# natir/br

Measured on AMD Instinct MI355X. Metric: corrected Gbases/sec at k=19, 10 kb ONT-error reads, higher is better.
Workload: dtype u64 k-mers / 1-bit set

## Files before the change

br_amd/csrc/brx_partbuild.hip:

```cpp
#include "brx_internal.hpp"
#include "brx_index.hpp"

#include <stdlib.h>
#include <string.h>

namespace brx {
uint64_t scan_tmp_bytes(uint32_t n);
int exclusive_scan_lens(const uint32_t *d_lens, uint32_t n, uint64_t *d_tmp, uint64_t *d_out_offsets,
                        unsigned long long *d_total, hipStream_t s);
}

using namespace brx;

namespace {

constexpr int F_BITS = 12;
constexpr int MAX_LEVELS = 4;
constexpr int MAX_DIGIT_BITS = 9;
static_assert(MAX_DIGIT_BITS <= 9, "the digit scans of the partition passes are written for at most 512 digits");

struct Plan {
    int k, nbits, nlev;
    int bits[MAX_LEVELS];
    int rem_in[MAX_LEVELS];
// ... 102 lines not shown
    const unsigned long long lo = x * R;
    unsigned long long hi = lo + R;
    if (hi > n_items)
        hi = n_items;
    return {lo + j, hi, (G - x + 7ull) >> 3};
}

struct L1Args {
    const uint8_t *bases;
    const uint64_t *offsets;
    uint32_t n_reads;
    uint64_t total;
    uint32_t n_items;
    int k, nbits, bits;
    uint32_t *matrix;
    const uint64_t *pos;
    uint32_t *keys_out;
    uint64_t out_cap;
};

__device__ __forceinline__ void l1_prepare(const L1Args &a, uint32_t item, uint32_t *pk, uint32_t *bnd, uint32_t *sh_r0,
                                           uint32_t &n_here, bool search)
{
    const uint64_t off0 = a.offsets[0];
    const uint64_t g0 = (uint64_t)item * L1_TILE;
    const uint64_t left = a.total - g0;
    n_here = (uint32_t)(left < L1_TILE ? left : L1_TILE);
    const uint32_t win = n_here + (uint32_t)a.k + 32u;
    pack_window(a.bases + off0, a.total, g0, win, pk);
    for (uint32_t w = threadIdx.x; w < BND_WORDS; w += 256)
        bnd[w] = 0;
// ... 37 lines not shown

struct L1Next {
    uint4 q0, q1;
    uint64_t off;
    uint32_t m[(1u << MAX_DIGIT_BITS) / 256u];
};

__device__ __forceinline__ uint32_t l1_window_words(const L1Args &a, uint32_t item, uint32_t &n_here)
{
    const uint64_t left = a.total - (uint64_t)item * L1_TILE;
    n_here = (uint32_t)(left < L1_TILE ? left : L1_TILE);
    return (n_here + (uint32_t)a.k + 32u + 15u) / 16u;
}

template <bool ROW>
__device__ __forceinline__ void l1_fetch(const L1Args &a, uint32_t item, uint32_t r_first, L1Next &nx)
{
    const uint64_t off0 = a.offsets[0];
    const uint8_t *bases = a.bases + off0;
    const uint64_t g0 = (uint64_t)item * L1_TILE;
    uint32_t n_here;
    const uint32_t nwords = l1_window_words(a, item, n_here);
    const uint64_t p0 = g0 + 16ull * threadIdx.x, p1 = p0 + 16ull * 256ull;
    nx.q0 = make_uint4(0, 0, 0, 0);
    nx.q1 = make_uint4(0, 0, 0, 0);
    if (threadIdx.x < nwords && p0 + 16 <= a.total)
        __builtin_memcpy(&nx.q0, bases + p0, 16);
    if (256u + threadIdx.x < nwords && p1 + 16 <= a.total)
        __builtin_memcpy(&nx.q1, bases + p1, 16);
    const uint32_t r = r_first + threadIdx.x;
    nx.off = a.offsets[r <= a.n_reads ? r : a.n_reads] - off0;
    if (ROW) {
        const uint32_t B = 1u << a.bits;
#pragma unroll
        for (uint32_t q = 0; q < (1u << MAX_DIGIT_BITS) / 256u; q++) {
            const uint32_t b = threadIdx.x + 256u * q;
            nx.m[q] = b < B ? a.matrix[(uint64_t)item * B + b] : 0u;
        }
    }
}

__device__ __forceinline__ uint32_t l1_pack16(const L1Args &a, const uint4 &q, uint64_t p)
{
    uint32_t v[4] = {q.x, q.y, q.z, q.w};
    if (p + 16 > a.total) {
        const uint8_t *bases = a.bases + a.offsets[0];
        v[0] = v[1] = v[2] = v[3] = 0;
        for (uint32_t j = 0; j < 16; j++)
            if (p + j < a.total)
                v[j >> 2] |= (uint32_t)bases[p + j] << (8u * (j & 3u));
    }
    return (pack4(v[0]) << 24) | (pack4(v[1]) << 16) | (pack4(v[2]) << 8) | pack4(v[3]);
}

__device__ __forceinline__ void l1_consume(const L1Args &a, uint32_t item, const L1Next &nx, uint32_t *pk, uint32_t *bnd, uint32_t *sh_r0,
                                           uint32_t &n_here, bool first)
{
    const uint64_t off0 = a.offsets[0];
    const uint64_t g0 = (uint64_t)item * L1_TILE;
    const uint32_t nwords = l1_window_words(a, item, n_here);
    if (threadIdx.x < nwords)
        pk[threadIdx.x] = l1_pack16(a, nx.q0, g0 + 16ull * threadIdx.x);
    if (256u + threadIdx.x < nwords)
        pk[256u + threadIdx.x] = l1_pack16(a, nx.q1, g0 + 16ull * (256u + threadIdx.x));
    for (uint32_t w = threadIdx.x; w < BND_WORDS; w += 256)
        bnd[w] = 0;
    if (threadIdx.x == 0 && !first) {
        sh_r0[0] += sh_r0[1];
        sh_r0[1] = 0;
    }
    __syncthreads();
    const uint64_t lim = g0 + n_here + (uint64_t)a.k;
    uint32_t before_next = 0;
    uint64_t o = nx.off;
    for (uint32_t r = sh_r0[0] + threadIdx.x; r <= a.n_reads; r += 256) {
        if (o >= lim)
            break;
        const uint32_t p = (uint32_t)(o - g0);
        atomicOr(&bnd[p >> 5], 1u << (p & 31u));
        before_next += o <= g0 + L1_TILE ? 1u : 0u;
        if (r + 256u <= a.n_reads)
            o = a.offsets[r + 256u] - off0;
    }
    if (before_next)
        atomicAdd(&sh_r0[1], before_next);
    __syncthreads();
}

__device__ __forceinline__ void l1_search(const L1Args &a, uint32_t item, uint32_t *sh_r0)
{
    if (threadIdx.x == 0) {
        const uint64_t off0 = a.offsets[0], g0 = (uint64_t)item * L1_TILE;
        uint32_t lo = 0, hi = a.n_reads + 1;
        while (lo < hi) {
            const uint32_t mid = lo + (hi - lo) / 2;
            if (a.offsets[mid] - off0 <= g0)
                lo = mid + 1;
            else
                hi = mid;
        }
        sh_r0[0] = lo;
        sh_r0[1] = 0;
    }
    __syncthreads();
}

__device__ __forceinline__ bool l1_valid(const uint32_t *bnd, uint32_t p, int k)
{
    const uint32_t q = p + 1u;
    const uint32_t w = q >> 5, sh = q & 31u;
    const uint64_t two = ((uint64_t)bnd[w + 1] << 32) | bnd[w];
    const uint32_t bits = (uint32_t)(two >> sh) & ((k > 1) ? ((1u << (k - 1)) - 1u) : 0u);
    return bits == 0u;
}

static_assert(L1_TILE == 256u * 16u, "l1_for_each_hash: 16 positions per thread");
template <int UNROLL = 4, typename F>
// ... 18 lines not shown
#pragma unroll UNROLL
    for (uint32_t j = 0; j < left; j++) {
        if ((vb & vmask) == 0ull)
            f(((popc64(fwd) & 1) ? rc : fwd) >> 1);
        const uint64_t b = next >> 62;
        next <<= 2;
        vb >>= 1;
        fwd = ((fwd << 2) | b) & mask;
        rc = (rc >> 2) | ((b ^ 2ull) << top);
    }
}

#ifndef BRX_L1HIST_WAVES
#define BRX_L1HIST_WAVES 1
#endif
__global__ __launch_bounds__(256, BRX_L1HIST_WAVES) void l1_hist_kernel(L1Args a)
{
    extern __shared__ uint32_t lds[];
    __shared__ uint32_t pk[PACK_WORDS];
    __shared__ uint32_t bnd[BND_WORDS];
    __shared__ uint32_t sh_r0[2];
    const uint32_t B = 1u << a.bits;
    const int shift = a.nbits - a.bits;
    uint32_t lo, hi;
    l1_range(a.n_items, lo, hi);
    if (lo >= hi)
        return;
    l1_search(a, lo, sh_r0);
    L1Next nx;
    l1_fetch<false>(a, lo, sh_r0[0], nx);
    for (uint32_t item = lo; item < hi; item++) {
        for (uint32_t b = threadIdx.x; b < B; b += 256)
            lds[b] = 0;
        uint32_t n_here;
        l1_consume(a, item, nx, pk, bnd, sh_r0, n_here, item == lo);
        if (item + 1 < hi)
            l1_fetch<false>(a, item + 1, sh_r0[0] + sh_r0[1], nx);
        l1_for_each_hash(pk, bnd, n_here, a.k, [&](uint64_t h) { atomicAdd(&lds[(uint32_t)(h >> shift)], 1u); });
        __syncthreads();
        for (uint32_t b = threadIdx.x; b < B; b += 256)
            a.matrix[(uint64_t)item * B + b] = lds[b];
        __syncthreads();
    }
}

__global__ __launch_bounds__(256) void col_scan_partial_kernel(const uint32_t *__restrict__ m, uint32_t n_items, uint32_t B, uint32_t CH,
                                                               uint64_t *__restrict__ part)
{
    const uint32_t chunk = blockIdx.x;
    const uint32_t lo = chunk * CH, hi = (lo + CH < n_items) ? lo + CH : n_items;
    for (uint32_t b = threadIdx.x; b < B; b += 256) {
        uint64_t sum = 0;
        for (uint32_t it = lo; it < hi; it++)
            sum += m[(uint64_t)it * B + b];
        part[(uint64_t)chunk * B + b] = sum;
    }
}

__global__ __launch_bounds__(256) void col_scan_columns_kernel(uint64_t *__restrict__ part, uint32_t n_chunks, uint32_t B,
                                                               uint64_t *__restrict__ coltot)
{
    __shared__ uint64_t wsum[4];
    const uint32_t b = blockIdx.x;
    const uint32_t per = (n_chunks + 255u) / 256u;
    const uint32_t c0 = threadIdx.x * per;
    uint64_t v[8];
    uint64_t mine = 0;
    for (uint32_t q = 0; q < per && q < 8u; q++) {
        const uint32_t c = c0 + q;
        v[q] = c < n_chunks ? part[(uint64_t)c * B + b] : 0;
        mine += v[q];
    }
    uint64_t incl = mine;
    for (int d = 1; d < 64; d <<= 1) {
        const uint64_t t = __shfl_up(incl, d);
        if ((threadIdx.x & 63) >= (unsigned)d)
            incl += t;
    }
    if ((threadIdx.x & 63) == 63)
        wsum[threadIdx.x >> 6] = incl;
    __syncthreads();
    uint64_t base = 0;
    for (uint32_t w = 0; w < (threadIdx.x >> 6); w++)
        base += wsum[w];
    uint64_t run = base + incl - mine;
    for (uint32_t q = 0; q < per && q < 8u; q++) {
        const uint32_t c = c0 + q;
        if (c < n_chunks)
            part[(uint64_t)c * B + b] = run;
        run += v[q];
    }
    if (threadIdx.x == 255)
        coltot[b] = base + incl;
}

__global__ __launch_bounds__(64) void col_scan_digits_kernel(const uint64_t *__restrict__ coltot, uint32_t B, uint64_t *__restrict__ coff,
                                                             unsigned long long *__restrict__ total)
{
    uint64_t carry = 0;
    for (uint32_t b0 = 0; b0 < B; b0 += 64) {
        const uint32_t b = b0 + threadIdx.x;
        const uint64_t v = b < B ? coltot[b] : 0;
        uint64_t incl = v;
        for (int d = 1; d < 64; d <<= 1) {
            const uint64_t t = __shfl_up(incl, d);
            if (threadIdx.x >= (unsigned)d)
                incl += t;
        }
        if (b < B)
            coff[b] = carry + incl - v;
        carry += __shfl(incl, 63);
    }
    if (threadIdx.x == 0) {
        coff[B] = carry;
        *total = carry;
    }
}

__global__ __launch_bounds__(256) void col_scan_positions_kernel(const uint32_t *__restrict__ m, uint32_t n_items, uint32_t B, uint32_t CH,
                                                                 const uint64_t *__restrict__ part, const uint64_t *__restrict__ coff,
                                                                 uint64_t *__restrict__ pos)
{
    const uint32_t chunk = blockIdx.x;
    const uint32_t lo = chunk * CH, hi = (lo + CH < n_items) ? lo + CH : n_items;
    for (uint32_t b = threadIdx.x; b < B; b += 256) {
        uint64_t run = part[(uint64_t)chunk * B + b] + coff[b];
        for (uint32_t it = lo; it < hi; it++) {
            pos[(uint64_t)it * B + b] = run;
            run += m[(uint64_t)it * B + b];
        }
    }
}

template <bool TABLE>
__global__ __launch_bounds__(256) void flat_insert_kernel(L1Args a, uint32_t *__restrict__ bits, uint64_t *__restrict__ lines,
                                                          uint32_t line_shift, uint32_t m, uint32_t w,
                                                          unsigned long long *__restrict__ n_new)
{
    __shared__ uint32_t pk[PACK_WORDS];
    __shared__ uint32_t bnd[BND_WORDS];
    __shared__ uint32_t sh_r0[2];
    uint32_t added = 0;
    uint32_t lo, hi;
    l1_range(a.n_items, lo, hi);
    for (uint32_t item = lo; item < hi; item++) {
// ... 7 lines not shown
                } else {
                    const uint64_t h = khash(kmer, a.k);
                    atomicOr(bits + (h >> 5), 1u << (h & 31u));
                }
            }
        __syncthreads();
    }
    if (TABLE) {
        for (int d = 32; d > 0; d >>= 1)
            added += __shfl_down(added, d);
        if ((threadIdx.x & 63) == 0 && added)
            atomicAdd(n_new, (unsigned long long)added);
    }
}

__device__ __forceinline__ void block_scan_bins(uint32_t B, const uint32_t *cntv, uint32_t *lofs, uint32_t *lcur, uint32_t *sh_wsum)
{
    const uint32_t BPT = (B + 255u) / 256u;
    uint32_t mine = 0;
    for (uint32_t q = 0; q < BPT; q++) {
        const uint32_t b = threadIdx.x * BPT + q;
        if (b < B)
            mine += cntv[b];
    }
    uint32_t incl = mine;
    for (int d = 1; d < 64; d <<= 1) {
        const uint32_t t = __shfl_up(incl, d);
        if ((threadIdx.x & 63) >= (unsigned)d)
            incl += t;
    }
    if ((threadIdx.x & 63) == 63)
        sh_wsum[threadIdx.x >> 6] = incl;
    __syncthreads();
    uint32_t wbase = 0;
    for (uint32_t w = 0; w < (threadIdx.x >> 6); w++)
        wbase += sh_wsum[w];
    uint32_t run = wbase + incl - mine;
    for (uint32_t q = 0; q < BPT; q++) {
        const uint32_t b = threadIdx.x * BPT + q;
        if (b < B) {
            lofs[b] = run;
            lcur[b] = run;
            run += cntv[b];
        }
    }
}

constexpr uint32_t L1_SECTOR = 8;
constexpr uint32_t L1_OWN = ((1u << MAX_DIGIT_BITS) + 255u) / 256u;

#ifndef BRX_L1SCAT_WAVES
#define BRX_L1SCAT_WAVES 5
#endif
__global__ __launch_bounds__(256, BRX_L1SCAT_WAVES) void l1_scatter_kernel(L1Args a)
{
    extern __shared__ __attribute__((aligned(16))) uint8_t lds_raw[];
    __shared__ uint32_t pk[PACK_WORDS];
    __shared__ uint32_t bnd[BND_WORDS];
    __shared__ uint32_t sh_r0[2];
    __shared__ uint32_t sh_wsum[4];
    const uint32_t T = L1_TILE;
    const uint32_t B = 1u << a.bits;
    uint32_t *stage_key = (uint32_t *)lds_raw;
    unsigned long long *gsm = (unsigned long long *)(stage_key + T);
    uint32_t *cntv = (uint32_t *)(gsm + B);
    uint32_t *lofs = cntv + B;
    uint32_t *lcur = lofs + B;
    const int shift = a.nbits - a.bits;
    const uint64_t child_mask = (1ull << shift) - 1ull;
    uint32_t lo, hi;
    l1_range(a.n_items, lo, hi);
    if (lo >= hi)
        return;
    for (uint32_t b = threadIdx.x; b < B; b += 256) {
        const unsigned long long p0 = a.pos[(uint64_t)lo * B + b];
        const unsigned long long ph = p0 & (L1_SECTOR - 1);
        gsm[b] = (p0 / L1_SECTOR) | (ph << 32) | (ph << 36);
    }
    uint32_t creg[L1_OWN][L1_SECTOR];
#pragma unroll
    for (uint32_t q = 0; q < L1_OWN; q++)
#pragma unroll
        for (uint32_t jj = 0; jj < L1_SECTOR; jj++)
            creg[q][jj] = 0;
    l1_search(a, lo, sh_r0);
    L1Next nx;
    l1_fetch<true>(a, lo, sh_r0[0], nx);
    for (uint32_t item = lo; item < hi; item++) {
#pragma unroll
        for (uint32_t q = 0; q < L1_OWN; q++)
            if (threadIdx.x + 256u * q < B)
                cntv[threadIdx.x + 256u * q] = nx.m[q];
        uint32_t n_here;
        l1_consume(a, item, nx, pk, bnd, sh_r0, n_here, item == lo);
        if (item + 1 < hi)
            l1_fetch<true>(a, item + 1, sh_r0[0] + sh_r0[1], nx);
        block_scan_bins(B, cntv, lofs, lcur, sh_wsum);
        __syncthreads();
        l1_for_each_hash<BRX_L1_UNROLL>(pk, bnd, n_here, a.k, [&](uint64_t h) {
            const uint32_t d = (uint32_t)(h >> shift);
            const uint32_t slot = atomicAdd(&lcur[d], 1u);
            stage_key[slot] = (uint32_t)(h & child_mask);
        });
        __syncthreads();
#pragma unroll
        for (uint32_t q = 0; q < L1_OWN; q++) {
            const uint32_t d = threadIdx.x + 256u * q;
            if (d < B) {
                const unsigned long long m = gsm[d];
                const uint32_t n = cntv[d], base = lofs[d];
                const uint32_t gsx = (uint32_t)m, cc = (uint32_t)(m >> 32) & 15u, ph = (uint32_t)(m >> 36) & 15u;
                const uint32_t tot = cc + n, full = tot / L1_SECTOR, r = tot % L1_SECTOR;
// ... 47 lines not shown
                    a.keys_out[g + jj] = creg[q][jj];
        }
    }
}

__global__ void tiles_from_offsets_kernel(const uint64_t *__restrict__ poff, uint64_t n_parents, uint32_t tile,
                                          uint32_t *__restrict__ ntiles)
{
    const uint64_t p = (uint64_t)blockIdx.x * blockDim.x + threadIdx.x;
    if (p >= n_parents)
        return;
    const uint64_t n = poff[p + 1] - poff[p];
    ntiles[p] = (uint32_t)((n + tile - 1) / tile);
}

__global__ void fill_item_parent_kernel(const uint64_t *__restrict__ item_off, uint64_t n_parents,
                                        uint32_t *__restrict__ item_parent)
{
    const uint64_t p = (uint64_t)blockIdx.x * blockDim.x + threadIdx.x;
    if (p >= n_parents)
        return;
    const uint64_t lo = item_off[p], hi = item_off[p + 1];
    for (uint64_t i = lo; i < hi; i++)
        item_parent[i] = (uint32_t)p;
}

struct LnArgs {
    const uint32_t *keys_in;
    const uint64_t *poff;
    uint64_t n_parents;
    const uint64_t *item_off;
    const uint32_t *item_parent;
    const unsigned long long *n_items;
    uint32_t tile;
    int rem_in, bits;
    uint32_t *matrix;
    const uint64_t *pos;
    void *keys_out;
    uint64_t in_cap, out_cap;
};

template <int KPT>
__device__ __forceinline__ uint32_t ln_load(const LnArgs &a, uint64_t parent, uint64_t t, uint32_t (&key)[KPT])
{
    const uint64_t lo = a.poff[parent] + t * a.tile;
    const uint64_t hi_p = a.poff[parent + 1];
    const uint64_t hi = (lo + a.tile < hi_p) ? lo + a.tile : hi_p;
    uint32_t cnt = 0;
#pragma unroll
    for (int q = 0; q < KPT; q++) {
        const uint64_t i = lo + (uint64_t)q * 256 + threadIdx.x;
        if (i < hi && store_ok(i, a.in_cap)) {
            key[q] = a.keys_in[i];
            cnt = q + 1;
        }
    }
    return cnt;
}

template <int KPT>
#ifndef BRX_LNHIST_WAVES
#define BRX_LNHIST_WAVES 1
#endif
__global__ __launch_bounds__(256, BRX_LNHIST_WAVES) void ln_hist_kernel(LnArgs a)
{
    extern __shared__ uint32_t lds[];
    const uint32_t B = 1u << a.bits;
    const int shift = a.rem_in - a.bits;
    const unsigned long long n_items = *a.n_items;
    const ItemRange ir = xcd_items(n_items);
    for (unsigned long long item = ir.first; item < ir.end; item += ir.step) {
        const uint64_t parent = a.item_parent[item];
        const uint64_t io = a.item_off[parent];
        const uint64_t t = item - io;
        for (uint32_t b = threadIdx.x; b < B; b += 256)
            lds[b] = 0;
        __syncthreads();
        uint32_t key[KPT];
        const uint32_t cnt = ln_load<KPT>(a, parent, t, key);
#pragma unroll
        for (int q = 0; q < KPT; q++)
            if ((uint32_t)q < cnt)
                atomicAdd(&lds[(key[q] >> shift) & (B - 1u)], 1u);
        __syncthreads();
        for (uint32_t b = threadIdx.x; b < B; b += 256)
            a.matrix[B * (io + t) + b] = lds[b];
        __syncthreads();
    }
}

__global__ __launch_bounds__(256) void ln_colscan_kernel(const uint32_t *__restrict__ m, const uint64_t *__restrict__ poff,
                                                         const uint64_t *__restrict__ item_off, uint64_t n_parents, uint32_t B,
                                                         uint64_t *__restrict__ pos, uint64_t *__restrict__ coff)
{
    __shared__ uint64_t wsum[4];
    for (uint64_t p = blockIdx.x; p < n_parents; p += gridDim.x) {
        const uint64_t io = item_off[p], nt = item_off[p + 1] - io;
        const uint32_t BPT = (B + 255u) / 256u;
        uint64_t tot[2] = {0, 0};
        for (uint64_t t = 0; t < nt; t++)
            for (uint32_t q = 0; q < BPT; q++) {
// ... 42 lines not shown
    extern __shared__ __attribute__((aligned(16))) uint8_t lds_raw[];
    __shared__ uint32_t sh_wsum[4];
    const uint32_t T = a.tile;
    const uint32_t B = 1u << a.bits;
    uint32_t *stage_key = (uint32_t *)lds_raw;
    uint16_t *stage_dig = (uint16_t *)(lds_raw + (size_t)T * 4);
    unsigned long long *gbase = (unsigned long long *)(lds_raw + (size_t)T * 6);
    uint32_t *cntv = (uint32_t *)(lds_raw + (size_t)T * 6 + (size_t)B * 8);
    uint32_t *lofs = cntv + B;
    uint32_t *lcur = lofs + B;
    const int shift = a.rem_in - a.bits;
    const uint32_t child_mask = (1u << shift) - 1u;
    OUT *out = (OUT *)a.keys_out;
    const unsigned long long n_items = *a.n_items;
    const ItemRange ir = xcd_items(n_items);
    for (unsigned long long item = ir.first; item < ir.end; item += ir.step) {
        const uint64_t parent = a.item_parent[item];
        const uint64_t io = a.item_off[parent];
        const uint64_t t = item - io;
        for (uint32_t b = threadIdx.x; b < B; b += 256) {
            const uint64_t mi = B * (io + t) + b;
            cntv[b] = a.matrix[mi];
            gbase[b] = a.pos[mi];
        }
        uint32_t key[KPT];
        const uint32_t cnt = ln_load<KPT>(a, parent, t, key);
        __syncthreads();
        block_scan_bins(B, cntv, lofs, lcur, sh_wsum);
        __syncthreads();
#pragma unroll
        for (int q = 0; q < KPT; q++)
            if ((uint32_t)q < cnt) {
                const uint32_t d = (key[q] >> shift) & (B - 1u);
                const uint32_t slot = atomicAdd(&lcur[d], 1u);
                stage_key[slot] = key[q] & child_mask;
                stage_dig[slot] = (uint16_t)d;
            }
        __syncthreads();
        const uint32_t n_tile = lofs[B - 1] + cntv[B - 1];
        for (uint32_t idx = threadIdx.x; idx < n_tile; idx += 256) {
            const uint32_t d = stage_dig[idx];
            const uint64_t at = gbase[d] + (idx - lofs[d]);
            if (store_ok(at, a.out_cap))
                out[at] = (OUT)stage_key[idx];
        }
        __syncthreads();
    }
}

constexpr int P3_WAVES = 4;
constexpr uint32_t F_SIZE = 1u << F_BITS;
constexpr uint32_t CNT_WORDS = F_SIZE / 2;
constexpr uint32_t BIT_WORDS = F_SIZE / 32;
constexpr uint32_t CHUNK_MAX = 65000;

constexpr uint32_t STAGE_KEYS = 704;

constexpr uint32_t EMIT_CAP = 256;

// ... 483 lines not shown
};

}

namespace brx {

struct PartState {
    Plan pl;
    Plan pl_wide;
    bool use_wide = false;
    std::vector<PartBatch> batches, spare;
    uint32_t *d_ntiles = nullptr;
    uint64_t ntiles_cap = 0;
    uint64_t *d_item_off = nullptr;
    uint64_t item_off_cap = 0;
    uint32_t *d_item_parent = nullptr;
    uint64_t item_parent_cap = 0;
    uint32_t *d_matrix = nullptr;
    uint64_t matrix_cap = 0;
    uint64_t *d_pos = nullptr;
    uint64_t pos_cap = 0;
    uint64_t *d_colpart = nullptr;
    uint64_t colpart_cap = 0;
    uint64_t *d_scan_tmp = nullptr;
    uint64_t scan_tmp_cap = 0;
    unsigned long long *d_scalars = nullptr;
    uint64_t *d_coff[MAX_LEVELS] = {nullptr, nullptr, nullptr, nullptr};
    uint32_t *d_keys_mid = nullptr;
    uint64_t keys_mid_cap = 0;
    uint32_t *d_keys_mid2 = nullptr;
    uint64_t keys_mid2_cap = 0;
    uint16_t *d_keys_fin = nullptr;
    uint64_t keys_fin_cap = 0;
    uint32_t *d_merged = nullptr;
    uint64_t merged_cap = 0;
    uint64_t *d_l1off_all = nullptr;
    uint32_t *d_cnts = nullptr;
    uint64_t *d_shift = nullptr;
// ... 102 lines not shown

void part_free(brx_counter *c)
{
    PartState *st = c->part;
    if (!st)
        return;
    for (auto *v : {&st->batches, &st->spare})
        for (auto &b : *v) {
            if (b.borrowed)
                continue;
            if (b.d_keys)
                (void)hipFree(b.d_keys);
            if (b.d_l1off)
                (void)hipFree(b.d_l1off);
        }
    for (void *p : {(void *)st->d_ntiles, (void *)st->d_item_off, (void *)st->d_item_parent, (void *)st->d_matrix,
                    (void *)st->d_pos, (void *)st->d_colpart, (void *)st->d_scan_tmp, (void *)st->d_scalars, (void *)st->d_coff[0],
                    (void *)st->d_coff[1], (void *)st->d_coff[2], (void *)st->d_coff[3], (void *)st->d_keys_mid,
                    (void *)st->d_keys_mid2, (void *)st->d_keys_fin,
                    (void *)st->d_merged, (void *)st->d_l1off_all, (void *)st->d_cnts, (void *)st->d_shift})
        if (p)
            (void)hipFree(p);
    delete st;
    c->part = nullptr;
}

int part_reset(brx_counter *c)
{
    PartState *st = c->part;
    for (auto &b : st->batches)
        if (!b.borrowed)
            st->spare.push_back(b);
// ... 24 lines not shown
int part_add_partitioned(brx_counter *c, const uint32_t *d_keys, const uint64_t *d_l1off, uint64_t n_keys)
{
    PartState *st = c->part;
    if (n_keys == 0)
        return BRX_OK;
    PartBatch b;
    b.d_keys = const_cast<uint32_t *>(d_keys);
    b.d_l1off = const_cast<uint64_t *>(d_l1off);
    b.n = n_keys;
    b.cap = n_keys;
    b.borrowed = true;
    st->batches.push_back(b);
    return BRX_OK;
}

static int ensure_matrix(PartState *st, uint64_t n_entries)
{
    uint64_t capb = st->matrix_cap;
    BRX_TRY(ensure_dev((void **)&st->d_matrix, &capb, (n_entries + 1) * 4));
    st->matrix_cap = capb;
    capb = st->pos_cap;
    BRX_TRY(ensure_dev((void **)&st->d_pos, &capb, (n_entries + 2) * 8));
    st->pos_cap = capb;
    capb = st->scan_tmp_cap;
    BRX_TRY(ensure_dev((void **)&st->d_scan_tmp, &capb, scan_tmp_bytes((uint32_t)n_entries) + 64));
    st->scan_tmp_cap = capb;
    return BRX_OK;
}

static size_t scatter_lds_bytes(uint32_t tile, int bits)
{
    const size_t B = (size_t)1 << bits;
    return (size_t)tile * 6 + B * 8 + B * 12 + 64;
}

static size_t l1_scatter_lds_bytes(int bits)
{
// ... 18 lines not shown
        }
    if (!b.d_keys) {
        uint64_t capb = 0;
        BRX_TRY(ensure_dev((void **)&b.d_keys, &capb, (max_keys + 1) * 4));
        b.cap = capb / 4;
        BRX_HIP(hipMalloc((void **)&b.d_l1off, (pl.nchild[0] + 1) * 8));
    }
    const uint32_t B = 1u << pl.bits[0];
    const uint64_t n_items64 = (total_bases + L1_TILE - 1) / L1_TILE;
    if (n_items64 * B >= (1ull << 32)) {
        set_error("batch of %llu bases is too large for one partition pass; split it", (unsigned long long)total_bases);
        return BRX_ERR_UNSUPPORTED;
    }
    const uint32_t n_items = (uint32_t)n_items64;
    const uint64_t n_entries = (uint64_t)B * n_items;
    BRX_TRY(ensure_matrix(st, n_entries));
    L1Args a;
    memset(&a, 0, sizeof(a));
    a.bases = d_bases;
    a.offsets = d_offsets;
    a.n_reads = n_reads;
    a.total = total_bases;
    a.n_items = n_items;
    a.k = pl.k;
    a.nbits = pl.nbits;
    a.bits = pl.bits[0];
    a.matrix = st->d_matrix;
    a.pos = st->d_pos;
    a.keys_out = b.d_keys;
    a.out_cap = b.cap;
    const char *genv = getenv("BRX_L1_GRID");
    const long gev = genv ? atol(genv) : 0;
    const uint32_t hist_blocks = gev > 0 ? (uint32_t)gev : 2048u, scatter_blocks = gev > 0 ? (uint32_t)gev : 2560u;
    const int grid = (int)(n_items < hist_blocks ? n_items : hist_blocks);
    {
        KernelTimer t("part_l1_hist", s);
        l1_hist_kernel<<<grid, 256, (size_t)B * 4, s>>>(a);
    }
    trace_stage(s, "partition level 1: histograms");
    {
        KernelTimer t("offsets_scan", s);
        uint32_t CH = 64;
        while ((n_items + CH - 1) / CH > 2048u)
            CH *= 2;
        const uint32_t n_chunks = (n_items + CH - 1) / CH;
        uint64_t capb = st->colpart_cap;
        BRX_TRY(ensure_dev((void **)&st->d_colpart, &capb, ((uint64_t)n_chunks + 1) * B * 8));
        st->colpart_cap = capb;
        uint64_t *coltot = st->d_colpart + (uint64_t)n_chunks * B;
        col_scan_partial_kernel<<<n_chunks, 256, 0, s>>>(st->d_matrix, n_items, B, CH, st->d_colpart);
        col_scan_columns_kernel<<<B, 256, 0, s>>>(st->d_colpart, n_chunks, B, coltot);
        col_scan_digits_kernel<<<1, 64, 0, s>>>(coltot, B, b.d_l1off, st->d_scalars + 1);
        col_scan_positions_kernel<<<n_chunks, 256, 0, s>>>(st->d_matrix, n_items, B, CH, st->d_colpart, b.d_l1off, st->d_pos);
    }
    {
        KernelTimer t("part_l1_scatter", s);
        const size_t lds1 = l1_scatter_lds_bytes(a.bits);
        if (lds1 > 64 * 1024)
            BRX_HIP(hipFuncSetAttribute((const void *)l1_scatter_kernel, hipFuncAttributeMaxDynamicSharedMemorySize, (int)lds1));
        const uint32_t sgrid = n_items < scatter_blocks ? n_items : scatter_blocks;
        l1_scatter_kernel<<<sgrid, 256, lds1, s>>>(a);
    }
    trace_stage(s, "partition level 1: scatter");
    BRX_HIP(hipGetLastError());
    unsigned long long tot = 0;
    BRX_HIP(hipMemcpyAsync(&tot, st->d_scalars + 1, 8, hipMemcpyDeviceToHost, s));
    BRX_HIP(hipStreamSynchronize(s));
    b.n = tot;
    st->batches.push_back(b);
    return BRX_OK;
}

template <typename OUT>
static int run_level(PartState *st, int l, const uint32_t *keys_in, const uint64_t *poff, uint64_t n_parents, uint64_t total,
                     void *keys_out, hipStream_t s, const char *tag_hist, const char *tag_scatter)
{
// ... 3 lines not shown
    const uint32_t tile = (pl.bits[l] > 8 || !small_tiles) ? 8192u : 4096u;
    const uint64_t ub_items = total / tile + n_parents + 1;
    const uint64_t n_entries = (uint64_t)B * ub_items;
    if (n_entries >= (1ull << 32)) {
        set_error("partition level %d needs %llu tile counters; split the input into smaller counters", l + 1,
                  (unsigned long long)n_entries);
        return BRX_ERR_UNSUPPORTED;
    }
    {
        uint64_t capb = st->ntiles_cap;
        BRX_TRY(ensure_dev((void **)&st->d_ntiles, &capb, (n_parents + 1) * 4));
        st->ntiles_cap = capb;
        capb = st->item_off_cap;
        BRX_TRY(ensure_dev((void **)&st->d_item_off, &capb, (n_parents + 2) * 8));
        st->item_off_cap = capb;
        capb = st->item_parent_cap;
        BRX_TRY(ensure_dev((void **)&st->d_item_parent, &capb, (ub_items + 1) * 4));
        st->item_parent_cap = capb;
    }
    BRX_TRY(ensure_matrix(st, n_entries > n_parents ? n_entries : n_parents));
    tiles_from_offsets_kernel<<<(unsigned)((n_parents + 255) / 256), 256, 0, s>>>(poff, n_parents, tile, st->d_ntiles);
    BRX_TRY(exclusive_scan_lens(st->d_ntiles, (uint32_t)n_parents, st->d_scan_tmp, st->d_item_off, st->d_scalars, s));
    fill_item_parent_kernel<<<(unsigned)((n_parents + 255) / 256), 256, 0, s>>>(st->d_item_off, n_parents, st->d_item_parent);
    trace_stage(s, tag_hist);
    BRX_HIP(hipMemsetAsync(st->d_matrix, 0, n_entries * 4, s));
    LnArgs a;
    memset(&a, 0, sizeof(a));
    a.keys_in = keys_in;
    a.in_cap = total;
    a.poff = poff;
    a.n_parents = n_parents;
    a.item_off = st->d_item_off;
    a.item_parent = st->d_item_parent;
    a.n_items = st->d_scalars;
    a.tile = tile;
    a.rem_in = pl.rem_in[l];
    a.bits = pl.bits[l];
    a.matrix = st->d_matrix;
    a.pos = st->d_pos;
    a.keys_out = keys_out;
    a.out_cap = total + 64;
    const int grid = 256 * 8;
    {
        KernelTimer t(tag_hist, s);
        if (tile == 8192u)
            ln_hist_kernel<32><<<grid, 256, (size_t)B * 4, s>>>(a);
        else
            ln_hist_kernel<16><<<grid, 256, (size_t)B * 4, s>>>(a);
// ... 43 lines not shown
                BRX_HIP(hipMalloc((void **)&dst->d_keylist_n, 8));
            BRX_HIP(hipMemsetAsync(dst->d_keylist_n, 0, 8, s));
            dst->keylist_valid = true;
        } else {
            BRX_HIP(hipMemsetAsync(dst->d_bits, 0, dst->nwords * 4, s));
            dst->bits_stale = false;
        }
        return BRX_OK;
    } else if (st->batches.size() == 1) {
        keys1 = st->batches[0].d_keys;
        l1off = st->batches[0].d_l1off;
    } else {
        uint64_t capb = st->merged_cap;
        BRX_TRY(ensure_dev((void **)&st->d_merged, &capb, (total + 1) * 4));
        st->merged_cap = capb;
        BRX_TRY(ensure_matrix(st, B1 + 1));
        BRX_HIP(hipMemsetAsync(st->d_cnts, 0, (uint64_t)B1 * 4, s));
        for (auto &b : st->batches)
            add_counts_kernel<<<(B1 + 255) / 256, 256, 0, s>>>(b.d_l1off, B1, st->d_cnts, nullptr);
        BRX_TRY(exclusive_scan_lens(st->d_cnts, B1, st->d_scan_tmp, st->d_l1off_all, st->d_scalars + 1, s));
        BRX_HIP(hipMemsetAsync(st->d_cnts, 0, (uint64_t)B1 * 4, s));
        for (auto &b : st->batches) {
            add_counts_kernel<<<(B1 + 255) / 256, 256, 0, s>>>(b.d_l1off, B1, st->d_cnts, st->d_shift);
            merge_segments_kernel<<<B1 < 4096u ? B1 : 4096u, 256, 0, s>>>(b.d_keys, b.d_l1off, st->d_l1off_all, st->d_shift, B1,
                                                                         st->d_merged);
        }
        keys1 = st->d_merged;
        l1off = st->d_l1off_all;
    }

    {
// ... 147 lines not shown
```

Measured before the change: 25.72.

## Fuse level-1 column scan into histogram ranges and prefetch next tiles

The level-1 histogram kernel now keeps per-block running column sums in registers and writes one row of range sums, and the scatter kernel uses the same block ranges. This replaces the separate partial and positions scan kernels and the full per-item position matrix. Boundary handling is restructured so each thread owns one read offset, and loads for the next tile are issued earlier to overlap with the hash work. The level-n pass precomputes per-item descriptors instead of parent lookups and prefetches the next item's rows and keys. The trade is more register pressure, and the scatter output now relies on the histogram and scatter grids having identical range splits.

```diff
diff --git a/br_amd/csrc/brx_partbuild.hip b/br_amd/csrc/brx_partbuild.hip
--- a/br_amd/csrc/brx_partbuild.hip
+++ b/br_amd/csrc/brx_partbuild.hip
@@ -140,7 +140,9 @@
     uint32_t n_items;
     int k, nbits, bits;
     uint32_t *matrix;
-    const uint64_t *pos;
+    uint32_t n_ranges;
+    uint64_t *rsum;
+    const uint64_t *coff;
     uint32_t *keys_out;
     uint64_t out_cap;
 };
@@ -208,9 +210,8 @@
 }
 
 template <bool ROW>
-__device__ __forceinline__ void l1_fetch(const L1Args &a, uint32_t item, uint32_t r_first, L1Next &nx)
-{
-    const uint64_t off0 = a.offsets[0];
+__device__ __forceinline__ void l1_fetch(const L1Args &a, uint64_t off0, uint32_t item, uint32_t r_first, L1Next &nx)
+{
     const uint8_t *bases = a.bases + off0;
     const uint64_t g0 = (uint64_t)item * L1_TILE;
     uint32_t n_here;
@@ -223,7 +224,7 @@
     if (256u + threadIdx.x < nwords && p1 + 16 <= a.total)
         __builtin_memcpy(&nx.q1, bases + p1, 16);
     const uint32_t r = r_first + threadIdx.x;
-    nx.off = a.offsets[r <= a.n_reads ? r : a.n_reads] - off0;
+    nx.off = a.offsets[r <= a.n_reads ? r : a.n_reads];
     if (ROW) {
         const uint32_t B = 1u << a.bits;
 #pragma unroll
@@ -234,11 +235,23 @@
     }
 }
 
-__device__ __forceinline__ uint32_t l1_pack16(const L1Args &a, const uint4 &q, uint64_t p)
+template <bool ROW>
+__device__ __forceinline__ void l1_landed(const L1Next &nx)
+{
+    asm volatile("" ::"v"(nx.q0.x), "v"(nx.q0.y), "v"(nx.q0.z), "v"(nx.q0.w), "v"(nx.q1.x), "v"(nx.q1.y), "v"(nx.q1.z), "v"(nx.q1.w),
+                 "v"(nx.off));
+    if (ROW) {
+#pragma unroll
+        for (uint32_t q = 0; q < (1u << MAX_DIGIT_BITS) / 256u; q++)
+            asm volatile("" ::"v"(nx.m[q]));
+    }
+}
+
+__device__ __forceinline__ uint32_t l1_pack16(const L1Args &a, uint64_t off0, const uint4 &q, uint64_t p)
 {
     uint32_t v[4] = {q.x, q.y, q.z, q.w};
     if (p + 16 > a.total) {
-        const uint8_t *bases = a.bases + a.offsets[0];
+        const uint8_t *bases = a.bases + off0;
         v[0] = v[1] = v[2] = v[3] = 0;
         for (uint32_t j = 0; j < 16; j++)
             if (p + j < a.total)
@@ -247,44 +260,48 @@
     return (pack4(v[0]) << 24) | (pack4(v[1]) << 16) | (pack4(v[2]) << 8) | pack4(v[3]);
 }
 
-__device__ __forceinline__ void l1_consume(const L1Args &a, uint32_t item, const L1Next &nx, uint32_t *pk, uint32_t *bnd, uint32_t *sh_r0,
-                                           uint32_t &n_here, bool first)
-{
-    const uint64_t off0 = a.offsets[0];
+__device__ __forceinline__ void l1_consume(const L1Args &a, uint64_t off0, uint32_t item, const L1Next &nx, uint32_t r_first, uint32_t *pk,
+                                           uint32_t *bnd, uint32_t *sh_r0, uint32_t &n_here)
+{
     const uint64_t g0 = (uint64_t)item * L1_TILE;
     const uint32_t nwords = l1_window_words(a, item, n_here);
     if (threadIdx.x < nwords)
-        pk[threadIdx.x] = l1_pack16(a, nx.q0, g0 + 16ull * threadIdx.x);
+        pk[threadIdx.x] = l1_pack16(a, off0, nx.q0, g0 + 16ull * threadIdx.x);
     if (256u + threadIdx.x < nwords)
-        pk[256u + threadIdx.x] = l1_pack16(a, nx.q1, g0 + 16ull * (256u + threadIdx.x));
+        pk[256u + threadIdx.x] = l1_pack16(a, off0, nx.q1, g0 + 16ull * (256u + threadIdx.x));
     for (uint32_t w = threadIdx.x; w < BND_WORDS; w += 256)
         bnd[w] = 0;
-    if (threadIdx.x == 0 && !first) {
-        sh_r0[0] += sh_r0[1];
+    const uint64_t lim = g0 + n_here + (uint64_t)a.k;
+    const uint32_t r = r_first + threadIdx.x;
+    const uint64_t o = nx.off - off0;
+    const bool mine = r <= a.n_reads && o < lim;
+    if (threadIdx.x == 0)
         sh_r0[1] = 0;
-    }
+    if (threadIdx.x == 255)
+        sh_r0[2] = mine ? 1u : 0u;
     __syncthreads();
-    const uint64_t lim = g0 + n_here + (uint64_t)a.k;
-    uint32_t before_next = 0;
-    uint64_t o = nx.off;
-    for (uint32_t r = sh_r0[0] + threadIdx.x; r <= a.n_reads; r += 256) {
-        if (o >= lim)
-            break;
-        const uint32_t p = (uint32_t)(o - g0);
+    if (mine) {
+        uint32_t p = (uint32_t)(o - g0);
         atomicOr(&bnd[p >> 5], 1u << (p & 31u));
-        before_next += o <= g0 + L1_TILE ? 1u : 0u;
-        if (r + 256u <= a.n_reads)
-            o = a.offsets[r + 256u] - off0;
-    }
-    if (before_next)
-        atomicAdd(&sh_r0[1], before_next);
-    __syncthreads();
-}
-
-__device__ __forceinline__ void l1_search(const L1Args &a, uint32_t item, uint32_t *sh_r0)
+        uint32_t before_next = o <= g0 + L1_TILE ? 1u : 0u;
+        if (sh_r0[2])
+            for (uint32_t r2 = r + 256u; r2 <= a.n_reads; r2 += 256u) {
+                const uint64_t o2 = a.offsets[r2] - off0;
+                if (o2 >= lim)
+                    break;
+                p = (uint32_t)(o2 - g0);
+                atomicOr(&bnd[p >> 5], 1u << (p & 31u));
+                before_next += o2 <= g0 + L1_TILE ? 1u : 0u;
+            }
+        if (before_next)
+            atomicAdd(&sh_r0[1], before_next);
+    }
+}
+
+__device__ __forceinline__ void l1_search(const L1Args &a, uint64_t off0, uint32_t item, uint32_t *sh_r0)
 {
     if (threadIdx.x == 0) {
-        const uint64_t off0 = a.offsets[0], g0 = (uint64_t)item * L1_TILE;
+        const uint64_t g0 = (uint64_t)item * L1_TILE;
         uint32_t lo = 0, hi = a.n_reads + 1;
         while (lo < hi) {
             const uint32_t mid = lo + (hi - lo) / 2;
@@ -294,7 +311,6 @@
                 hi = mid;
         }
         sh_r0[0] = lo;
-        sh_r0[1] = 0;
     }
     __syncthreads();
 }
@@ -343,62 +359,85 @@
 #ifndef BRX_L1HIST_WAVES
 #define BRX_L1HIST_WAVES 1
 #endif
+constexpr uint32_t L1_OWN = ((1u << MAX_DIGIT_BITS) + 255u) / 256u;
+
 __global__ __launch_bounds__(256, BRX_L1HIST_WAVES) void l1_hist_kernel(L1Args a)
 {
     extern __shared__ uint32_t lds[];
     __shared__ uint32_t pk[PACK_WORDS];
     __shared__ uint32_t bnd[BND_WORDS];
-    __shared__ uint32_t sh_r0[2];
+    __shared__ uint32_t sh_r0[3];
     const uint32_t B = 1u << a.bits;
     const int shift = a.nbits - a.bits;
     uint32_t lo, hi;
     l1_range(a.n_items, lo, hi);
-    if (lo >= hi)
-        return;
-    l1_search(a, lo, sh_r0);
-    L1Next nx;
-    l1_fetch<false>(a, lo, sh_r0[0], nx);
-    for (uint32_t item = lo; item < hi; item++) {
+    uint64_t rs[L1_OWN];
+#pragma unroll
+    for (uint32_t q = 0; q < L1_OWN; q++)
+        rs[q] = 0;
+    if (lo < hi) {
+        const uint64_t off0 = a.offsets[0];
+        l1_search(a, off0, lo, sh_r0);
+        uint32_t r_first = sh_r0[0];
+        L1Next nx;
+        l1_fetch<false>(a, off0, lo, r_first, nx);
         for (uint32_t b = threadIdx.x; b < B; b += 256)
             lds[b] = 0;
         uint32_t n_here;
-        l1_consume(a, item, nx, pk, bnd, sh_r0, n_here, item == lo);
-        if (item + 1 < hi)
-            l1_fetch<false>(a, item + 1, sh_r0[0] + sh_r0[1], nx);
-        l1_for_each_hash(pk, bnd, n_here, a.k, [&](uint64_t h) { atomicAdd(&lds[(uint32_t)(h >> shift)], 1u); });
+        l1_landed<false>(nx);
+        l1_consume(a, off0, lo, nx, r_first, pk, bnd, sh_r0, n_here);
         __syncthreads();
-        for (uint32_t b = threadIdx.x; b < B; b += 256)
-            a.matrix[(uint64_t)item * B + b] = lds[b];
-        __syncthreads();
-    }
-}
-
-__global__ __launch_bounds__(256) void col_scan_partial_kernel(const uint32_t *__restrict__ m, uint32_t n_items, uint32_t B, uint32_t CH,
-                                                               uint64_t *__restrict__ part)
-{
-    const uint32_t chunk = blockIdx.x;
-    const uint32_t lo = chunk * CH, hi = (lo + CH < n_items) ? lo + CH : n_items;
-    for (uint32_t b = threadIdx.x; b < B; b += 256) {
-        uint64_t sum = 0;
-        for (uint32_t it = lo; it < hi; it++)
-            sum += m[(uint64_t)it * B + b];
-        part[(uint64_t)chunk * B + b] = sum;
-    }
-}
-
-__global__ __launch_bounds__(256) void col_scan_columns_kernel(uint64_t *__restrict__ part, uint32_t n_chunks, uint32_t B,
+        r_first += sh_r0[1];
+        l1_fetch<false>(a, off0, lo + 1 < hi ? lo + 1 : lo, r_first, nx);
+        for (uint32_t item = lo; item < hi; item++) {
+            l1_for_each_hash(pk, bnd, n_here, a.k, [&](uint64_t h) { atomicAdd(&lds[(uint32_t)(h >> shift)], 1u); });
+            __syncthreads();
+            uint32_t row[L1_OWN];
+#pragma unroll
+            for (uint32_t q = 0; q < L1_OWN; q++) {
+                const uint32_t b = threadIdx.x + 256u * q;
+                row[q] = 0;
+                if (b < B) {
+                    row[q] = lds[b];
+                    lds[b] = 0;
+                }
+            }
+            l1_landed<false>(nx);
+            if (item + 1 < hi) {
+                l1_consume(a, off0, item + 1, nx, r_first, pk, bnd, sh_r0, n_here);
+                __syncthreads();
+                r_first += sh_r0[1];
+            }
+#pragma unroll
+            for (uint32_t q = 0; q < L1_OWN; q++) {
+                const uint32_t b = threadIdx.x + 256u * q;
+                if (b < B)
+                    a.matrix[(uint64_t)item * B + b] = row[q];
+                rs[q] += row[q];
+            }
+            l1_fetch<false>(a, off0, item + 2 < hi ? item + 2 : hi - 1, r_first, nx);
+        }
+    }
+#pragma unroll
+    for (uint32_t q = 0; q < L1_OWN; q++) {
+        const uint32_t b = threadIdx.x + 256u * q;
+        if (b < B && store_ok((uint64_t)blockIdx.x * B + b, (uint64_t)a.n_ranges * B))
+            a.rsum[(uint64_t)blockIdx.x * B + b] = rs[q];
+    }
+}
+
+__global__ __launch_bounds__(256) void col_scan_columns_kernel(uint64_t *__restrict__ part, uint32_t n_rows, uint32_t B,
                                                                uint64_t *__restrict__ coltot)
 {
     __shared__ uint64_t wsum[4];
     const uint32_t b = blockIdx.x;
-    const uint32_t per = (n_chunks + 255u) / 256u;
+    const uint32_t per = (n_rows + 255u) / 256u;
     const uint32_t c0 = threadIdx.x * per;
-    uint64_t v[8];
     uint64_t mine = 0;
-    for (uint32_t q = 0; q < per && q < 8u; q++) {
+    for (uint32_t q = 0; q < per; q++) {
         const uint32_t c = c0 + q;
-        v[q] = c < n_chunks ? part[(uint64_t)c * B + b] : 0;
-        mine += v[q];
+        if (c < n_rows)
+            mine += part[(uint64_t)c * B + b];
     }
     uint64_t incl = mine;
     for (int d = 1; d < 64; d <<= 1) {
@@ -413,11 +452,13 @@
     for (uint32_t w = 0; w < (threadIdx.x >> 6); w++)
         base += wsum[w];
     uint64_t run = base + incl - mine;
-    for (uint32_t q = 0; q < per && q < 8u; q++) {
+    for (uint32_t q = 0; q < per; q++) {
         const uint32_t c = c0 + q;
-        if (c < n_chunks)
+        if (c < n_rows) {
+            const uint64_t v = part[(uint64_t)c * B + b];
             part[(uint64_t)c * B + b] = run;
-        run += v[q];
+            run += v;
+        }
     }
     if (threadIdx.x == 255)
         coltot[b] = base + incl;
@@ -443,21 +484,6 @@
     if (threadIdx.x == 0) {
         coff[B] = carry;
         *total = carry;
-    }
-}
-
-__global__ __launch_bounds__(256) void col_scan_positions_kernel(const uint32_t *__restrict__ m, uint32_t n_items, uint32_t B, uint32_t CH,
-                                                                 const uint64_t *__restrict__ part, const uint64_t *__restrict__ coff,
-                                                                 uint64_t *__restrict__ pos)
-{
-    const uint32_t chunk = blockIdx.x;
-    const uint32_t lo = chunk * CH, hi = (lo + CH < n_items) ? lo + CH : n_items;
-    for (uint32_t b = threadIdx.x; b < B; b += 256) {
-        uint64_t run = part[(uint64_t)chunk * B + b] + coff[b];
-        for (uint32_t it = lo; it < hi; it++) {
-            pos[(uint64_t)it * B + b] = run;
-            run += m[(uint64_t)it * B + b];
-        }
     }
 }
 
@@ -495,16 +521,16 @@
     }
 }
 
-__device__ __forceinline__ void block_scan_bins(uint32_t B, const uint32_t *cntv, uint32_t *lofs, uint32_t *lcur, uint32_t *sh_wsum)
+__device__ __forceinline__ void scan_bins_begin(uint32_t B, const uint32_t *cntv, uint32_t *sh_wsum, uint32_t &mine, uint32_t &incl)
 {
     const uint32_t BPT = (B + 255u) / 256u;
-    uint32_t mine = 0;
+    mine = 0;
     for (uint32_t q = 0; q < BPT; q++) {
         const uint32_t b = threadIdx.x * BPT + q;
         if (b < B)
             mine += cntv[b];
     }
-    uint32_t incl = mine;
+    incl = mine;
     for (int d = 1; d < 64; d <<= 1) {
         const uint32_t t = __shfl_up(incl, d);
         if ((threadIdx.x & 63) >= (unsigned)d)
@@ -512,7 +538,12 @@
     }
     if ((threadIdx.x & 63) == 63)
         sh_wsum[threadIdx.x >> 6] = incl;
-    __syncthreads();
+}
+
+__device__ __forceinline__ void scan_bins_end(uint32_t B, const uint32_t *cntv, uint32_t *lofs, uint32_t *lcur, const uint32_t *sh_wsum,
+                                              uint32_t mine, uint32_t incl)
+{
+    const uint32_t BPT = (B + 255u) / 256u;
     uint32_t wbase = 0;
     for (uint32_t w = 0; w < (threadIdx.x >> 6); w++)
         wbase += sh_wsum[w];
@@ -527,8 +558,15 @@
     }
 }
 
+__device__ __forceinline__ void block_scan_bins(uint32_t B, const uint32_t *cntv, uint32_t *lofs, uint32_t *lcur, uint32_t *sh_wsum)
+{
+    uint32_t mine, incl;
+    scan_bins_begin(B, cntv, sh_wsum, mine, incl);
+    __syncthreads();
+    scan_bins_end(B, cntv, lofs, lcur, sh_wsum, mine, incl);
+}
+
 constexpr uint32_t L1_SECTOR = 8;
-constexpr uint32_t L1_OWN = ((1u << MAX_DIGIT_BITS) + 255u) / 256u;
 
 #ifndef BRX_L1SCAT_WAVES
 #define BRX_L1SCAT_WAVES 5
@@ -538,7 +576,7 @@
     extern __shared__ __attribute__((aligned(16))) uint8_t lds_raw[];
     __shared__ uint32_t pk[PACK_WORDS];
     __shared__ uint32_t bnd[BND_WORDS];
-    __shared__ uint32_t sh_r0[2];
+    __shared__ uint32_t sh_r0[3];
     __shared__ uint32_t sh_wsum[4];
     const uint32_t T = L1_TILE;
     const uint32_t B = 1u << a.bits;
@@ -554,7 +592,7 @@
     if (lo >= hi)
         return;
     for (uint32_t b = threadIdx.x; b < B; b += 256) {
-        const unsigned long long p0 = a.pos[(uint64_t)lo * B + b];
+        const unsigned long long p0 = a.coff[b] + a.rsum[(uint64_t)blockIdx.x * B + b];
         const unsigned long long ph = p0 & (L1_SECTOR - 1);
         gsm[b] = (p0 / L1_SECTOR) | (ph << 32) | (ph << 36);
     }
@@ -564,19 +602,25 @@
 #pragma unroll
         for (uint32_t jj = 0; jj < L1_SECTOR; jj++)
             creg[q][jj] = 0;
-    l1_search(a, lo, sh_r0);
+    const uint64_t off0 = a.offsets[0];
+    l1_search(a, off0, lo, sh_r0);
+    uint32_t r_first = sh_r0[0];
     L1Next nx;
-    l1_fetch<true>(a, lo, sh_r0[0], nx);
+    l1_fetch<true>(a, off0, lo, r_first, nx);
     for (uint32_t item = lo; item < hi; item++) {
+        l1_landed<true>(nx);
 #pragma unroll
         for (uint32_t q = 0; q < L1_OWN; q++)
             if (threadIdx.x + 256u * q < B)
                 cntv[threadIdx.x + 256u * q] = nx.m[q];
         uint32_t n_here;
-        l1_consume(a, item, nx, pk, bnd, sh_r0, n_here, item == lo);
-        if (item + 1 < hi)
-            l1_fetch<true>(a, item + 1, sh_r0[0] + sh_r0[1], nx);
-        block_scan_bins(B, cntv, lofs, lcur, sh_wsum);
+        l1_consume(a, off0, item, nx, r_first, pk, bnd, sh_r0, n_here);
+        uint32_t mine, incl;
+        scan_bins_begin(B, cntv, sh_wsum, mine, incl);
+        __syncthreads();
+        r_first += sh_r0[1];
+        scan_bins_end(B, cntv, lofs, lcur, sh_wsum, mine, incl);
+        l1_fetch<true>(a, off0, item + 1 < hi ? item + 1 : item, r_first, nx);
         __syncthreads();
         l1_for_each_hash<BRX_L1_UNROLL>(pk, bnd, n_here, a.k, [&](uint64_t h) {
             const uint32_t d = (uint32_t)(h >> shift);
@@ -654,23 +698,33 @@
     ntiles[p] = (uint32_t)((n + tile - 1) / tile);
 }
 
-__global__ void fill_item_parent_kernel(const uint64_t *__restrict__ item_off, uint64_t n_parents,
-                                        uint32_t *__restrict__ item_parent)
+struct LnItem {
+    uint64_t lo;
+    uint32_t n;
+    uint32_t pad;
+};
+
+__global__ void fill_items_kernel(const uint64_t *__restrict__ poff, const uint64_t *__restrict__ item_off, uint64_t n_parents,
+                                  uint32_t tile, LnItem *__restrict__ items)
 {
     const uint64_t p = (uint64_t)blockIdx.x * blockDim.x + threadIdx.x;
     if (p >= n_parents)
         return;
-    const uint64_t lo = item_off[p], hi = item_off[p + 1];
-    for (uint64_t i = lo; i < hi; i++)
-        item_parent[i] = (uint32_t)p;
+    const uint64_t i0 = item_off[p], i1 = item_off[p + 1];
+    const uint64_t k1 = poff[p + 1];
+    uint64_t k = poff[p];
+    for (uint64_t i = i0; i < i1; i++, k += tile) {
+        LnItem it;
+        it.lo = k;
+        it.n = (uint32_t)(k1 - k < tile ? k1 - k : tile);
+        it.pad = 0;
+        items[i] = it;
+    }
 }
 
 struct LnArgs {
     const uint32_t *keys_in;
-    const uint64_t *poff;
-    uint64_t n_parents;
-    const uint64_t *item_off;
-    const uint32_t *item_parent;
+    const LnItem *items;
     const unsigned long long *n_items;
     uint32_t tile;
     int rem_in, bits;
@@ -680,22 +734,35 @@
     uint64_t in_cap, out_cap;
 };
 
+__device__ __forceinline__ uint4 ln_item_load(const LnArgs &a, unsigned long long item)
+{
+    return *reinterpret_cast<const uint4 *>(a.items + item);
+}
+
+__device__ __forceinline__ LnItem ln_item_get(const uint4 &v)
+{
+    LnItem it;
+    it.lo = ((uint64_t)(uint32_t)__builtin_amdgcn_readfirstlane((int)v.y) << 32) | (uint32_t)__builtin_amdgcn_readfirstlane((int)v.x);
+    it.n = (uint32_t)__builtin_amdgcn_readfirstlane((int)v.z);
+    it.pad = 0;
+    return it;
+}
+
 template <int KPT>
-__device__ __forceinline__ uint32_t ln_load(const LnArgs &a, uint64_t parent, uint64_t t, uint32_t (&key)[KPT])
-{
-    const uint64_t lo = a.poff[parent] + t * a.tile;
-    const uint64_t hi_p = a.poff[parent + 1];
-    const uint64_t hi = (lo + a.tile < hi_p) ? lo + a.tile : hi_p;
-    uint32_t cnt = 0;
+__device__ __forceinline__ void ln_load(const LnArgs &a, const LnItem &it, uint32_t (&key)[KPT])
+{
 #pragma unroll
     for (int q = 0; q < KPT; q++) {
-        const uint64_t i = lo + (uint64_t)q * 256 + threadIdx.x;
-        if (i < hi && store_ok(i, a.in_cap)) {
+        const uint32_t j = (uint32_t)q * 256u + threadIdx.x;
+        const uint64_t i = it.lo + (j < it.n ? j : 0u);
+        if (store_ok(i, a.in_cap))
             key[q] = a.keys_in[i];
-            cnt = q + 1;
-        }
-    }
-    return cnt;
+    }
+}
+
+__device__ __forceinline__ uint32_t ln_count(const LnItem &it)
+{
+    return it.n > threadIdx.x ? (it.n - threadIdx.x + 255u) / 256u : 0u;
 }
 
 template <int KPT>
@@ -709,22 +776,26 @@
     const int shift = a.rem_in - a.bits;
     const unsigned long long n_items = *a.n_items;
     const ItemRange ir = xcd_items(n_items);
+    if (ir.first >= ir.end)
+        return;
+    uint4 it_raw = ln_item_load(a, ir.first);
     for (unsigned long long item = ir.first; item < ir.end; item += ir.step) {
-        const uint64_t parent = a.item_parent[item];
-        const uint64_t io = a.item_off[parent];
-        const uint64_t t = item - io;
+        const LnItem it = ln_item_get(it_raw);
+        uint32_t key[KPT];
+        ln_load<KPT>(a, it, key);
+        const uint32_t cnt = ln_count(it);
+        const unsigned long long next = item + ir.step;
+        it_raw = ln_item_load(a, next < ir.end ? next : item);
         for (uint32_t b = threadIdx.x; b < B; b += 256)
             lds[b] = 0;
         __syncthreads();
-        uint32_t key[KPT];
-        const uint32_t cnt = ln_load<KPT>(a, parent, t, key);
 #pragma unroll
         for (int q = 0; q < KPT; q++)
             if ((uint32_t)q < cnt)
                 atomicAdd(&lds[(key[q] >> shift) & (B - 1u)], 1u);
         __syncthreads();
         for (uint32_t b = threadIdx.x; b < B; b += 256)
-            a.matrix[B * (io + t) + b] = lds[b];
+            a.matrix[B * item + b] = lds[b];
         __syncthreads();
     }
 }
@@ -797,17 +868,33 @@
     OUT *out = (OUT *)a.keys_out;
     const unsigned long long n_items = *a.n_items;
     const ItemRange ir = xcd_items(n_items);
+    if (ir.first >= ir.end)
+        return;
+    constexpr uint32_t OWN = ((1u << MAX_DIGIT_BITS) + 255u) / 256u;
+    auto load_rows = [&](unsigned long long item, uint32_t(&rc)[OWN], uint64_t(&rp)[OWN]) {
+#pragma unroll
+        for (uint32_t q = 0; q < OWN; q++) {
+            const uint32_t b = threadIdx.x + 256u * q;
+            const uint64_t mi = B * item + (b < B ? b : 0u);
+            rc[q] = a.matrix[mi];
+            rp[q] = a.pos[mi];
+        }
+    };
+    LnItem it = ln_item_get(ln_item_load(a, ir.first));
+    uint32_t key[KPT], rc[OWN];
+    uint64_t rp[OWN];
+    load_rows(ir.first, rc, rp);
+    ln_load<KPT>(a, it, key);
     for (unsigned long long item = ir.first; item < ir.end; item += ir.step) {
-        const uint64_t parent = a.item_parent[item];
-        const uint64_t io = a.item_off[parent];
-        const uint64_t t = item - io;
-        for (uint32_t b = threadIdx.x; b < B; b += 256) {
-            const uint64_t mi = B * (io + t) + b;
-            cntv[b] = a.matrix[mi];
-            gbase[b] = a.pos[mi];
-        }
-        uint32_t key[KPT];
-        const uint32_t cnt = ln_load<KPT>(a, parent, t, key);
+#pragma unroll
+        for (uint32_t q = 0; q < OWN; q++) {
+            const uint32_t b = threadIdx.x + 256u * q;
+            if (b < B) {
+                cntv[b] = rc[q];
+                gbase[b] = rp[q];
+            }
+        }
+        const uint32_t cnt = ln_count(it);
         __syncthreads();
         block_scan_bins(B, cntv, lofs, lcur, sh_wsum);
         __syncthreads();
@@ -826,6 +913,12 @@
             const uint64_t at = gbase[d] + (idx - lofs[d]);
             if (store_ok(at, a.out_cap))
                 out[at] = (OUT)stage_key[idx];
+        }
+        const unsigned long long next = item + ir.step;
+        if (next < ir.end) {
+            it = ln_item_get(ln_item_load(a, next));
+            load_rows(next, rc, rp);
+            ln_load<KPT>(a, it, key);
         }
         __syncthreads();
     }
@@ -1339,14 +1432,12 @@
     uint64_t ntiles_cap = 0;
     uint64_t *d_item_off = nullptr;
     uint64_t item_off_cap = 0;
-    uint32_t *d_item_parent = nullptr;
-    uint64_t item_parent_cap = 0;
+    LnItem *d_items = nullptr;
+    uint64_t items_cap = 0;
     uint32_t *d_matrix = nullptr;
     uint64_t matrix_cap = 0;
     uint64_t *d_pos = nullptr;
     uint64_t pos_cap = 0;
-    uint64_t *d_colpart = nullptr;
-    uint64_t colpart_cap = 0;
     uint64_t *d_scan_tmp = nullptr;
     uint64_t scan_tmp_cap = 0;
     unsigned long long *d_scalars = nullptr;
@@ -1479,8 +1570,8 @@
             if (b.d_l1off)
                 (void)hipFree(b.d_l1off);
         }
-    for (void *p : {(void *)st->d_ntiles, (void *)st->d_item_off, (void *)st->d_item_parent, (void *)st->d_matrix,
-                    (void *)st->d_pos, (void *)st->d_colpart, (void *)st->d_scan_tmp, (void *)st->d_scalars, (void *)st->d_coff[0],
+    for (void *p : {(void *)st->d_ntiles, (void *)st->d_item_off, (void *)st->d_items, (void *)st->d_matrix,
+                    (void *)st->d_pos, (void *)st->d_scan_tmp, (void *)st->d_scalars, (void *)st->d_coff[0],
                     (void *)st->d_coff[1], (void *)st->d_coff[2], (void *)st->d_coff[3], (void *)st->d_keys_mid,
                     (void *)st->d_keys_mid2, (void *)st->d_keys_fin,
                     (void *)st->d_merged, (void *)st->d_l1off_all, (void *)st->d_cnts, (void *)st->d_shift})
@@ -1535,13 +1626,13 @@
     return BRX_OK;
 }
 
-static int ensure_matrix(PartState *st, uint64_t n_entries)
+static int ensure_matrix(PartState *st, uint64_t n_entries, uint64_t n_pos)
 {
     uint64_t capb = st->matrix_cap;
     BRX_TRY(ensure_dev((void **)&st->d_matrix, &capb, (n_entries + 1) * 4));
     st->matrix_cap = capb;
     capb = st->pos_cap;
-    BRX_TRY(ensure_dev((void **)&st->d_pos, &capb, (n_entries + 2) * 8));
+    BRX_TRY(ensure_dev((void **)&st->d_pos, &capb, (n_pos + 2) * 8));
     st->pos_cap = capb;
     capb = st->scan_tmp_cap;
     BRX_TRY(ensure_dev((void **)&st->d_scan_tmp, &capb, scan_tmp_bytes((uint32_t)n_entries) + 64));
@@ -1590,7 +1681,12 @@
     }
     const uint32_t n_items = (uint32_t)n_items64;
     const uint64_t n_entries = (uint64_t)B * n_items;
-    BRX_TRY(ensure_matrix(st, n_entries));
+    const char *genv = getenv("BRX_L1_GRID");
+    const long gev = genv ? atol(genv) : 0;
+    const uint32_t want_ranges = gev > 0 ? (uint32_t)gev : 2560u;
+    const uint32_t n_ranges = n_items < want_ranges ? n_items : want_ranges;
+    BRX_TRY(ensure_matrix(st, n_entries, ((uint64_t)n_ranges + 1) * B));
+    uint64_t *coltot = st->d_pos + (uint64_t)n_ranges * B;
     L1Args a;
     memset(&a, 0, sizeof(a));
     a.bases = d_bases;
@@ -1602,40 +1698,27 @@
     a.nbits = pl.nbits;
     a.bits = pl.bits[0];
     a.matrix = st->d_matrix;
-    a.pos = st->d_pos;
+    a.n_ranges = n_ranges;
+    a.rsum = st->d_pos;
+    a.coff = b.d_l1off;
     a.keys_out = b.d_keys;
     a.out_cap = b.cap;
-    const char *genv = getenv("BRX_L1_GRID");
-    const long gev = genv ? atol(genv) : 0;
-    const uint32_t hist_blocks = gev > 0 ? (uint32_t)gev : 2048u, scatter_blocks = gev > 0 ? (uint32_t)gev : 2560u;
-    const int grid = (int)(n_items < hist_blocks ? n_items : hist_blocks);
     {
         KernelTimer t("part_l1_hist", s);
-        l1_hist_kernel<<<grid, 256, (size_t)B * 4, s>>>(a);
+        l1_hist_kernel<<<n_ranges, 256, (size_t)B * 4, s>>>(a);
     }
     trace_stage(s, "partition level 1: histograms");
     {
         KernelTimer t("offsets_scan", s);
-        uint32_t CH = 64;
-        while ((n_items + CH - 1) / CH > 2048u)
-            CH *= 2;
-        const uint32_t n_chunks = (n_items + CH - 1) / CH;
-        uint64_t capb = st->colpart_cap;
-        BRX_TRY(ensure_dev((void **)&st->d_colpart, &capb, ((uint64_t)n_chunks + 1) * B * 8));
-        st->colpart_cap = capb;
-        uint64_t *coltot = st->d_colpart + (uint64_t)n_chunks * B;
-        col_scan_partial_kernel<<<n_chunks, 256, 0, s>>>(st->d_matrix, n_items, B, CH, st->d_colpart);
-        col_scan_columns_kernel<<<B, 256, 0, s>>>(st->d_colpart, n_chunks, B, coltot);
+        col_scan_columns_kernel<<<B, 256, 0, s>>>(st->d_pos, n_ranges, B, coltot);
         col_scan_digits_kernel<<<1, 64, 0, s>>>(coltot, B, b.d_l1off, st->d_scalars + 1);
-        col_scan_positions_kernel<<<n_chunks, 256, 0, s>>>(st->d_matrix, n_items, B, CH, st->d_colpart, b.d_l1off, st->d_pos);
     }
     {
         KernelTimer t("part_l1_scatter", s);
         const size_t lds1 = l1_scatter_lds_bytes(a.bits);
         if (lds1 > 64 * 1024)
             BRX_HIP(hipFuncSetAttribute((const void *)l1_scatter_kernel, hipFuncAttributeMaxDynamicSharedMemorySize, (int)lds1));
-        const uint32_t sgrid = n_items < scatter_blocks ? n_items : scatter_blocks;
-        l1_scatter_kernel<<<sgrid, 256, lds1, s>>>(a);
+        l1_scatter_kernel<<<n_ranges, 256, lds1, s>>>(a);
     }
     trace_stage(s, "partition level 1: scatter");
     BRX_HIP(hipGetLastError());
@@ -1669,24 +1752,21 @@
         capb = st->item_off_cap;
         BRX_TRY(ensure_dev((void **)&st->d_item_off, &capb, (n_parents + 2) * 8));
         st->item_off_cap = capb;
-        capb = st->item_parent_cap;
-        BRX_TRY(ensure_dev((void **)&st->d_item_parent, &capb, (ub_items + 1) * 4));
-        st->item_parent_cap = capb;
-    }
-    BRX_TRY(ensure_matrix(st, n_entries > n_parents ? n_entries : n_parents));
+        capb = st->items_cap;
+        BRX_TRY(ensure_dev((void **)&st->d_items, &capb, (ub_items + 1) * sizeof(LnItem)));
+        st->items_cap = capb;
+    }
+    BRX_TRY(ensure_matrix(st, n_entries > n_parents ? n_entries : n_parents, n_entries > n_parents ? n_entries : n_parents));
     tiles_from_offsets_kernel<<<(unsigned)((n_parents + 255) / 256), 256, 0, s>>>(poff, n_parents, tile, st->d_ntiles);
     BRX_TRY(exclusive_scan_lens(st->d_ntiles, (uint32_t)n_parents, st->d_scan_tmp, st->d_item_off, st->d_scalars, s));
-    fill_item_parent_kernel<<<(unsigned)((n_parents + 255) / 256), 256, 0, s>>>(st->d_item_off, n_parents, st->d_item_parent);
+    fill_items_kernel<<<(unsigned)((n_parents + 255) / 256), 256, 0, s>>>(poff, st->d_item_off, n_parents, tile, st->d_items);
     trace_stage(s, tag_hist);
     BRX_HIP(hipMemsetAsync(st->d_matrix, 0, n_entries * 4, s));
     LnArgs a;
     memset(&a, 0, sizeof(a));
     a.keys_in = keys_in;
     a.in_cap = total;
-    a.poff = poff;
-    a.n_parents = n_parents;
-    a.item_off = st->d_item_off;
-    a.item_parent = st->d_item_parent;
+    a.items = st->d_items;
     a.n_items = st->d_scalars;
     a.tile = tile;
     a.rem_in = pl.rem_in[l];
@@ -1760,7 +1840,7 @@
         uint64_t capb = st->merged_cap;
         BRX_TRY(ensure_dev((void **)&st->d_merged, &capb, (total + 1) * 4));
         st->merged_cap = capb;
-        BRX_TRY(ensure_matrix(st, B1 + 1));
+        BRX_TRY(ensure_matrix(st, B1 + 1, B1 + 1));
         BRX_HIP(hipMemsetAsync(st->d_cnts, 0, (uint64_t)B1 * 4, s));
         for (auto &b : st->batches)
             add_counts_kernel<<<(B1 + 255) / 256, 256, 0, s>>>(b.d_l1off, B1, st->d_cnts, nullptr);
```

New measurement: 26.26 (median of 6 runs). 1.02x the previous value.
